# XiaRho/CMDA

Hardware: AMD Instinct MI355X
Metric: training images/sec (512x512 image+event, MiT-B5) (higher is better)
Workload: dtype bf16

## Files before the change

cmda_amd/csrc/batchnorm.hip:

```cpp
#include "common.h"

namespace {

constexpr int kRowUnroll = 4;
constexpr int kBnSlots = CMDA_BN_SLOTS;

template <typename T>
__global__ void bn_reduce_kernel(const T* __restrict__ x, float* __restrict__ ws, long M, int C, int rows_per_block) {
  __shared__ float red[2][4][64][4];
  const int cx = threadIdx.x & 63, ry = threadIdx.x >> 6;
  const int c = (blockIdx.x * 64 + cx) * 4;
  x += (long)blockIdx.z * M * C;
  ws += (long)blockIdx.z * (kBnSlots + 1) * 2 * C;
  const long r0 = (long)blockIdx.y * rows_per_block, r1 = min(M, r0 + rows_per_block);
  float s[4] = {0, 0, 0, 0}, q[4] = {0, 0, 0, 0};
  if (c < C) {
    float sh[4];
    ld4(x + c, sh);
    for (long r = r0 + ry; r < r1; r += 4 * kRowUnroll) {
      float v[kRowUnroll][4];
#pragma unroll
      for (int u = 0; u < kRowUnroll; ++u) {
        const long ru = r + 4 * u;
        ld4(x + (ru < r1 ? ru : r) * C + c, v[u]);
// ... 276 lines not shown
    for (int u = 0; u < kRowUnroll; ++u) {
      const long ru = r + 4 * u;
      if (ru >= r1) break;
#pragma unroll
      for (int j = 0; j < 4; ++j) {
        const float xh = (v[u][j] - mu[j]) * rs[j];
        float dj = d[u][j];
        if (relu && xh * g[j] + b[j] <= 0.f) dj = 0.f;
        v[u][j] = g[j] * rs[j] * (dj - a1[j] - xh * a2[j]);
      }
      st4(dx + ru * C + c, v[u]);
    }
  }
}

static inline int rows_per_block(long M, int gx) {
  int rpb = 512;
  while (rpb > 32 && (M + rpb - 1) / rpb * gx < 1024) rpb >>= 1;
  return rpb;
}
static inline int rows_per_block_apply(long M, int gx) {
  int rpb = 256;
  while (rpb > 16 && (M + rpb - 1) / rpb * gx < 2048) rpb >>= 1;
  return rpb;
}
}

extern "C" int64_t cmda_bn_ws_floats(int C) { return (int64_t)(kBnSlots + 1) * 2 * C; }

extern "C" int cmda_bn_train_fwd(const void* x, const float* gamma, const float* beta, void* y, float* mean, float* rstd,
                                 float* running_mean, float* running_var, float* ws, int64_t M, int C, float eps,
                                 float momentum, int relu, int ldy, int coff, int groups, const int* order, int ws_has_stats,
                                 int dtype, void* stream) {
  if (M <= 0 || C <= 0) return CMDA_OK;
  if ((C & 3) || (ldy & 3) || (coff & 3) || groups < 1 || groups > 8) return CMDA_ERR_SHAPE;
  BnOrder ord;
  for (int i = 0; i < 8; ++i) ord.g[i] = (order && i < groups) ? order[i] : i;
  unsigned seen = 0;
  for (int i = 0; i < groups; ++i) {
    if (ord.g[i] < 0 || ord.g[i] >= groups) return CMDA_ERR_SHAPE;
    seen |= 1u << ord.g[i];
  }
  if (ws_has_stats && seen != (1u << groups) - 1u) return CMDA_ERR_SHAPE;
  if (!ws_has_stats) cmda_zero_async(ws, sizeof(float) * (size_t)groups * (kBnSlots + 1) * 2 * C, stream);
  const int gx = (C / 4 + 63) / 64;
  const int rpb = rows_per_block(M * groups, gx);
  dim3 rgrid(gx, (unsigned)((M + rpb - 1) / rpb), groups);
  const int arpb = rows_per_block_apply(M * groups, gx);
  dim3 agrid(gx, (unsigned)((M + arpb - 1) / arpb), groups);
  CMDA_DISPATCH_DTYPE(dtype, {
    if (!ws_has_stats) CMDA_LAUNCH((bn_reduce_kernel<T>), rgrid, dim3(256), 0, stream, (const T*)x, ws, (long)M, C, rpb);
    CMDA_LAUNCH((bn_finalize_kernel<T>), dim3((C + 7) / 8), dim3(256), 0, stream, (const T*)x, ws, mean, rstd,
                running_mean, running_var, (long)M, C, eps, momentum, groups, ord, ws_has_stats);
    CMDA_LAUNCH((bn_apply_kernel<T>), agrid, dim3(256), 0, stream, (const T*)x, mean, rstd, gamma, beta, (T*)y + coff, (long)M,
                C, relu, ldy, 0, arpb);
  });
  CMDA_CHECK_LAUNCH();
}

extern "C" int cmda_bn_train_fwd2(const void* x, int x_dtype, const float* gamma, const float* beta, void* y, int y_dtype,
                                  float* mean, float* rstd, float* running_mean, float* running_var, float* ws, int64_t M, int C,
                                  float eps, float momentum, int relu, int ldy, int coff, int groups, const int* order,
                                  const float* res32, void* y2_bf16, int ws_has_stats, void* stream) {
  if (M <= 0 || C <= 0) return CMDA_OK;
  if ((C & 3) || (ldy & 3) || (coff & 3) || groups < 1 || groups > 8) return CMDA_ERR_SHAPE;
  if ((x_dtype != CMDA_F32 && x_dtype != CMDA_BF16) || (y_dtype != CMDA_F32 && y_dtype != CMDA_BF16)) return CMDA_ERR_DTYPE;
  BnOrder ord;
  for (int i = 0; i < 8; ++i) ord.g[i] = (order && i < groups) ? order[i] : i;
  unsigned seen = 0;
  for (int i = 0; i < groups; ++i) {
    if (ord.g[i] < 0 || ord.g[i] >= groups) return CMDA_ERR_SHAPE;
    seen |= 1u << ord.g[i];
  }
  if (ws_has_stats && seen != (1u << groups) - 1u) return CMDA_ERR_SHAPE;
  if (!ws_has_stats) cmda_zero_async(ws, sizeof(float) * (size_t)groups * (kBnSlots + 1) * 2 * C, stream);
  const int gx = (C / 4 + 63) / 64;
  const int rpb = rows_per_block(M * groups, gx);
  dim3 rgrid(gx, (unsigned)((M + rpb - 1) / rpb), groups);
  const int arpb = rows_per_block_apply(M * groups, gx);
  dim3 agrid(gx, (unsigned)((M + arpb - 1) / arpb), groups);
#define CMDA_BN2_APPLY(TX, TY)                                                                                                    \
  CMDA_LAUNCH((bn_apply2_kernel<TX, TY>), agrid, dim3(256), 0, stream, (const TX*)x, mean, rstd, gamma, beta, (TY*)y + coff,      \
              res32, (bf16_t*)y2_bf16, (long)M, C, relu, ldy, arpb)
  CMDA_DISPATCH_DTYPE(x_dtype, {
    if (!ws_has_stats) CMDA_LAUNCH((bn_reduce_kernel<T>), rgrid, dim3(256), 0, stream, (const T*)x, ws, (long)M, C, rpb);
    CMDA_LAUNCH((bn_finalize_kernel<T>), dim3((C + 7) / 8), dim3(256), 0, stream, (const T*)x, ws, mean, rstd,
                running_mean, running_var, (long)M, C, eps, momentum, groups, ord, ws_has_stats);
    if (y_dtype == CMDA_F32) CMDA_BN2_APPLY(T, float); else CMDA_BN2_APPLY(T, bf16_t);
  });
#undef CMDA_BN2_APPLY
  CMDA_CHECK_LAUNCH();
}

extern "C" int cmda_bn_apply(const void* x, const float* mean, const float* rstd, const float* gamma, const float* beta,
                             void* y, int64_t M, int C, int relu, int ldy, int coff, int dtype, void* stream) {
  if (M <= 0 || C <= 0) return CMDA_OK;
  if ((C & 3) || (ldy & 3) || (coff & 3)) return CMDA_ERR_SHAPE;
  const int gx = (C / 4 + 63) / 64;
  const int arpb = rows_per_block_apply(M, gx);
  dim3 agrid(gx, (unsigned)((M + arpb - 1) / arpb));
  CMDA_DISPATCH_DTYPE(dtype, CMDA_LAUNCH((bn_apply_kernel<T>), agrid, dim3(256), 0, stream, (const T*)x, mean, rstd, gamma,
                                         beta, (T*)y, (long)M, C, relu, ldy, coff, arpb));
  CMDA_CHECK_LAUNCH();
}

extern "C" int cmda_bn_train_bwd(const void* dy, const void* x, const float* mean, const float* rstd, const float* gamma,
                                 const float* beta, void* dx, float* dgamma, float* dbeta, float* ws, int64_t M, int C,
                                 int relu, int lddy, int coff, int groups, int dtype, void* stream) {
// ... 18 lines not shown
```

cmda_amd/csrc/gemm_pp.hip:

```cpp
#include "gemm_kernels.h"

namespace {

typedef __attribute__((ext_vector_type(16))) float f32x16;

#ifndef CMDA_EMU
static __device__ __forceinline__ f32x16 mfma_bf16_32x32x16(u16x8 a, u16x8 b, f32x16 c) {
  return __builtin_amdgcn_mfma_f32_32x32x16_bf16(__builtin_bit_cast(bfx8, a), __builtin_bit_cast(bfx8, b), c, 0, 0, 0);
}
static __device__ __forceinline__ void raw_barrier() { __builtin_amdgcn_s_barrier(); }
static __device__ __forceinline__ void sched_fence() { __builtin_amdgcn_sched_barrier(0); }
static __device__ __forceinline__ void prio(int hi) {
  if (hi) __builtin_amdgcn_s_setprio(1);
  else __builtin_amdgcn_s_setprio(0);
}
static __device__ __forceinline__ void wait_lds() { asm volatile("s_waitcnt lgkmcnt(0)" ::: "memory"); }
static __device__ __forceinline__ void wait_dma_lds() { asm volatile("s_waitcnt vmcnt(0) lgkmcnt(0)" ::: "memory"); }
#else
static inline f32x16 mfma_bf16_32x32x16(u16x8 a, u16x8 b, f32x16 c) {
  auto& w = emu::my_wave();
  const int l = emu::my_lane();
  for (int j = 0; j < 8; ++j) { w.fa[l][j] = bf2f(a[j]); w.fb[l][j] = bf2f(b[j]); }
  emu::wave_barrier();
  const int col = l & 31, h = l >> 5;
  f32x16 d = c;
  for (int r = 0; r < 16; ++r) {
    const int row = (r & 3) + 8 * (r >> 2) + 4 * h;
    float acc = d[r];
    for (int hh = 0; hh < 2; ++hh)
      for (int j = 0; j < 8; ++j) acc = fmaf(w.fa[32 * hh + row][j], w.fb[32 * hh + col][j], acc);
    d[r] = acc;
  }
  emu::wave_barrier();
  return d;
}
static inline void raw_barrier() { __syncthreads(); }
static inline void sched_fence() {}
static inline void prio(int) {}
static inline void wait_lds() {}
static inline void wait_dma_lds() { emu::wave_barrier(); }
#endif

#ifdef CMDA_PP_TIMING
__device__ unsigned long long g_pp_stamps[2 * 4 * 4 * 4];
#define PP_STAMP(i) do { if (lane == 0 && (wid & 3) == 0 && blockIdx.x == 7 && kt >= 8 && kt < 12) \
    g_pp_stamps[((grp * 4 + (kt - 8)) * 4 + q) * 4 + (i)] = __builtin_amdgcn_s_memtime(); } while (0)
#else
#define PP_STAMP(i) do { } while (0)
#endif

constexpr int PP_BM = 256, PP_BN = 256, PP_BK = 64, PP_NW = 8;
constexpr int PP_SZ = PP_BM * PP_BK;
constexpr int PP_PITCH_C = PP_BN + 8;
constexpr size_t PP_LDS = (size_t)PP_BM * PP_PITCH_C * 2;

template <int ACT>
static __device__ __forceinline__ float pp_act(float x) {
  if (ACT == 1) return fmaxf(x, 0.f);
  if (ACT == 2) return gelu_erf(x);
  if (ACT == 3) return tanhf(x);
  return x;
}

template <bool BKS, bool ACONV, bool FAST = false>
__global__ __launch_bounds__(512, 1) void gemm_pp_kernel(GemmParams p) {
  typedef bf16_t T;
  __shared__ __attribute__((aligned(1024))) char smem[PP_LDS];
  T* const sAbase = reinterpret_cast<T*>(smem);
  T* const sBbase = sAbase + 2 * PP_SZ;

  const int tid = threadIdx.x, lane = tid & 63;
#ifndef CMDA_EMU
  const int wid = __builtin_amdgcn_readfirstlane(tid >> 6);
#else
  const int wid = tid >> 6;
#endif
  const int grp = wid >> 2, wc = wid & 3;
  const int l31 = lane & 31, h = lane >> 5;

  const int tiles_n = (p.N + PP_BN - 1) / PP_BN;
  const int ntile = gridDim.x;
  int bt = blockIdx.x;
  {
    const int q = ntile / 8, rr = ntile % 8, xcd = bt % 8, loc = bt / 8;
    bt = (xcd < rr ? xcd * (q + 1) : rr * (q + 1) + (xcd - rr) * q) + loc;
  }
  long mt, nt;
  {
    constexpr int GM = 4;
    const int tiles_m = (int)((p.M + PP_BM - 1) / PP_BM);
    if (tiles_n >= 2 * GM && tiles_m >= GM) {
      const int gsz = GM * tiles_n, gid = bt / gsz, first = gid * GM;
      const int gm = min(tiles_m - first, GM), r = bt - gid * gsz;
      mt = first + r % gm;
      nt = r / gm;
    } else {
      mt = bt / tiles_n;
      nt = bt % tiles_n;
    }
  }
  const long m0 = mt * PP_BM, n0 = nt * PP_BN;
  const int z = blockIdx.z;
  const int batch = z / p.batch2, batch2 = z - batch * p.batch2;
  const int nkt = (p.K + PP_BK - 1) / PP_BK;
  const T* baseA = reinterpret_cast<const T*>(p.A.ptr) + (long)batch * p.A.batch_stride + (long)batch2 * p.A.batch2_stride;
  const T* baseB = reinterpret_cast<const T*>(p.B.ptr) + (long)batch * p.B.batch_stride + (long)batch2 * p.B.batch2_stride;

  DmaSrc<false, PP_BM, ACONV, PP_NW, 1, 64, DmaMode<false, ACONV, FAST>::value> dA;
  DmaSrc<BKS, PP_BN, false, PP_NW, 1, 64, DmaMode<BKS, false, FAST>::value> dB;
  dA.init(p.A, baseA, wid, lane, m0, 0);
  dB.init(p.B, baseB, wid, lane, n0, 0);
  bool cellA = false;
  auto piece = [&](int stage, int kt, int i) {
    if (i == 0) cellA = dA.cell_begin(kt, 0);
    if (i < 4) glds16(dA.get(p.A, baseA, i, kt, cellA), reinterpret_cast<char*>(sAbase + stage * PP_SZ) + (wid * 4 + i) * 1024);
    else glds16(dB.get(p.B, baseB, i - 4, kt, false), reinterpret_cast<char*>(sBbase + stage * PP_SZ) + (wid * 4 + (i - 4)) * 1024);
  };

  f32x16 acc[4][2];
#pragma unroll
  for (int i = 0; i < 4; ++i)
#pragma unroll
    for (int j = 0; j < 2; ++j)
#pragma unroll
      for (int r = 0; r < 16; ++r) acc[i][j][r] = 0.f;

  auto load_a = [&](const T* sA, int mh, u16x8 (&fa)[2][4]) {
#pragma unroll
    for (int i = 0; i < 2; ++i) {
      const int row = grp * 128 + (mh * 2 + i) * 32 + l31;
#pragma unroll
      for (int s = 0; s < 4; ++s) fa[i][s] = *reinterpret_cast<const u16x8*>(&sA[row * PP_BK + (((2 * s + h) ^ ((row >> 1) & 7)) << 3)]);
    }
  };
  auto load_b = [&](const T* sB, int nh, u16x8 (&fb)[4]) {
    if constexpr (!BKS) {
      const int row = wc * 64 + nh * 32 + l31;
#pragma unroll
      for (int s = 0; s < 4; ++s) fb[s] = *reinterpret_cast<const u16x8*>(&sB[row * PP_BK + (((2 * s + h) ^ ((row >> 1) & 7)) << 3)]);
    } else {
      const int gi = lane >> 4, li = lane & 15, q = li >> 2, pp = li & 3;
      const int colbase = wc * 64 + nh * 32 + 16 * (gi & 1);
      const int cidx = (colbase >> 3) + (pp >> 1), half = (pp & 1) << 2;
#pragma unroll
      for (int s = 0; s < 4; ++s) {
        const int k0 = 16 * s + 8 * (gi >> 1) + q, k1 = k0 + 4;
        const u16x4 lo = lds_read_tr16(&sB[k0 * PP_BN + ((cidx ^ (k0 & 7)) << 3) + half]);
        const u16x4 hi = lds_read_tr16(&sB[k1 * PP_BN + ((cidx ^ (k1 & 7)) << 3) + half]);
        fb[s] = u16x8{lo[0], lo[1], lo[2], lo[3], hi[0], hi[1], hi[2], hi[3]};
      }
    }
  };

#pragma unroll
  for (int i = 0; i < 8; ++i) piece(0, 0, i);
  wait_dma_lds();
  raw_barrier();
  if (grp == 1) raw_barrier();

  u16x8 fa[2][4], fb[2][4];
  for (int kt = 0; kt < nkt; ++kt) {
    const int st = kt & 1;
    const T* sA = sAbase + st * PP_SZ;
    const T* sB = sBbase + st * PP_SZ;
    const bool more = kt + 1 < nkt;
#pragma unroll
    for (int q = 0; q < 4; ++q) {
      const int mh = q >> 1, nh = (q == 1 || q == 2) ? 1 : 0;
      PP_STAMP(0);
      if (q == 0 || q == 2) load_a(sA, mh, fa);
      if (q < 2) load_b(sB, nh, fb[nh]);
      if (more) {
        if (q == 0) { piece(st ^ 1, kt + 1, 0); piece(st ^ 1, kt + 1, 4); }
        if (q == 1) { piece(st ^ 1, kt + 1, 1); piece(st ^ 1, kt + 1, 2); piece(st ^ 1, kt + 1, 5); piece(st ^ 1, kt + 1, 6); }
        if (q == 2) { piece(st ^ 1, kt + 1, 3); piece(st ^ 1, kt + 1, 7); }
      }
      if (q == 3 && grp == 1) wait_dma_lds();
      if (q == 3 && grp == 0) wait_lds();
      sched_fence();
      raw_barrier();
      wait_lds();
      PP_STAMP(1);
      sched_fence();
      prio(1);
#pragma unroll
      for (int s = 0; s < 4; ++s)
#pragma unroll
        for (int i = 0; i < 2; ++i) acc[mh * 2 + i][nh] = mfma_bf16_32x32x16(fb[nh][s], fa[i][s], acc[mh * 2 + i][nh]);
      prio(0);
      PP_STAMP(2);
      if (q == 3 && grp == 0) wait_dma_lds();
      sched_fence();
      raw_barrier();
      PP_STAMP(3);
    }
  }
  if (grp == 0) raw_barrier();
  __syncthreads();

  T* sC = reinterpret_cast<T*>(smem);
  const float alpha = p.alpha;
  const int act = p.act;
#pragma unroll
  for (int j = 0; j < 2; ++j)
#pragma unroll
    for (int rg = 0; rg < 4; ++rg) {
      const int nl = wc * 64 + j * 32 + 8 * rg + 4 * h;
      float bv[4] = {0.f, 0.f, 0.f, 0.f};
      if (p.bias) {
#pragma unroll
        for (int e = 0; e < 4; ++e)
          if (n0 + nl + e < p.N) bv[e] = p.bias[n0 + nl + e];
      }
#pragma unroll
      for (int i = 0; i < 4; ++i) {
        const int ml = grp * 128 + i * 32 + l31;
        float v[4];
#pragma unroll
        for (int e = 0; e < 4; ++e) v[e] = alpha * acc[i][j][rg * 4 + e] + bv[e];
        if (act == 1) {
#pragma unroll
          for (int e = 0; e < 4; ++e) v[e] = pp_act<1>(v[e]);
        } else if (act == 2) {
#pragma unroll
          for (int e = 0; e < 4; ++e) v[e] = pp_act<2>(v[e]);
        } else if (act == 3) {
#pragma unroll
          for (int e = 0; e < 4; ++e) v[e] = pp_act<3>(v[e]);
        }
        st4(&sC[ml * PP_PITCH_C + nl], v);
      }
    }
  __syncthreads();
  const long cb = (long)batch * p.c_batch_stride + (long)batch2 * p.c_batch2_stride;
  T* C = reinterpret_cast<T*>(p.C) + cb;
  const bool vec = p.c_vec_ok != 0 && (p.ldc & 7) == 0 && ((reinterpret_cast<uintptr_t>(C) & 15) == 0);
  const bool stats = p.colstats != nullptr;
  float cs[8] = {0.f, 0.f, 0.f, 0.f, 0.f, 0.f, 0.f, 0.f}, cq[8] = {0.f, 0.f, 0.f, 0.f, 0.f, 0.f, 0.f, 0.f};
#pragma unroll 4
  for (int it = 0; it < (PP_BM * PP_BN / 8) / 512; ++it) {
    const int idx = it * 512 + tid;
    const int row = idx >> 5, ch = idx & 31;
    const long m = m0 + row, n = n0 + ch * 8;
// ... 20 lines not shown
    }
  }
  if (stats) {
#pragma unroll
    for (int e = 0; e < 8; ++e) {
      cs[e] += __shfl_xor(cs[e], 32, 64);
      cq[e] += __shfl_xor(cq[e], 32, 64);
    }
    __syncthreads();
    float* scr = reinterpret_cast<float*>(smem);
    const int wv = tid >> 6, ln = tid & 63;
    if (ln < 32) {
#pragma unroll
      for (int e = 0; e < 8; ++e) {
        scr[wv * 2 * PP_BN + ln * 8 + e] = cs[e];
        scr[wv * 2 * PP_BN + PP_BN + ln * 8 + e] = cq[e];
      }
    }
    __syncthreads();
    static_assert(2 * PP_BN == 512, "one thread per (statistic, column)");
    const int col = tid & (PP_BN - 1);
    if (n0 + col < p.N) {
      float t = 0.f;
#pragma unroll
      for (int w = 0; w < 8; ++w) t += scr[w * 2 * PP_BN + tid];
      const long gidx = (unsigned)m0 / (unsigned)p.colstats_rows;
      const unsigned slot = (unsigned)(m0 >> 6) & (CMDA_BN_SLOTS - 1);
      atomicAdd(p.colstats + (gidx * (CMDA_BN_SLOTS + 1) + slot) * 2 * (long)p.N + (tid < PP_BN ? 0 : p.N) + n0 + col, t);
    }
  }
}

}

#ifdef CMDA_PP_TIMING
extern "C" int cmda_debug_pp_stamps(unsigned long long* host_out) {
  return hipMemcpyFromSymbol(host_out, HIP_SYMBOL(g_pp_stamps), sizeof(unsigned long long) * 128) == hipSuccess ? 0 : -3;
}
#endif

int cmda_gemm_pp_(const cmda_gemm_params_t& p, void* stream) {
  const long tiles = (long)((p.M + PP_BM - 1) / PP_BM) * ((p.N + PP_BN - 1) / PP_BN);
  const long zz = (long)p.batch * p.batch2;
  if (tiles > 0x7fffffffL || zz > 65535) return CMDA_ERR_SHAPE;
  const dim3 grid((unsigned)tiles, 1, (unsigned)zz), blk(512);
  const bool bks = p.b_kstrided != 0, ac = p.A.conv == 1;
  if (p.a_kstrided || p.B.conv == 1) return CMDA_ERR_UNSUPPORTED;
  const bool nofast = p.tile_hint > 0 && (p.tile_hint & 2048);
  typedef DmaSrc<false, PP_BM, false, PP_NW, 1, 64, 1> FA;
  typedef DmaSrc<false, PP_BM, true, PP_NW, 1, 64, 2> FAC;
  typedef DmaSrc<false, PP_BN, false, PP_NW, 1, 64, 1> FB;
  typedef DmaSrc<true, PP_BN, false, PP_NW, 1, 64, 1> FBK;
  if (!bks && !ac) {
    if (!nofast && FA::mode_ok(p.A, 1) && FB::mode_ok(p.B, 1)) CMDA_LAUNCH((gemm_pp_kernel<false, false, true>), grid, blk, 0, stream, p);
    else CMDA_LAUNCH((gemm_pp_kernel<false, false, false>), grid, blk, 0, stream, p);
  } else if (!bks && ac) {
    if (!nofast && FAC::mode_ok(p.A, 2) && FB::mode_ok(p.B, 1)) CMDA_LAUNCH((gemm_pp_kernel<false, true, true>), grid, blk, 0, stream, p);
    else CMDA_LAUNCH((gemm_pp_kernel<false, true, false>), grid, blk, 0, stream, p);
  } else if (bks && !ac) {
    if (!nofast && FA::mode_ok(p.A, 1) && FBK::mode_ok(p.B, 1)) CMDA_LAUNCH((gemm_pp_kernel<true, false, true>), grid, blk, 0, stream, p);
    else CMDA_LAUNCH((gemm_pp_kernel<true, false, false>), grid, blk, 0, stream, p);
  }
  else return CMDA_ERR_UNSUPPORTED;
  CMDA_CHECK_LAUNCH();
}
```

cmda_amd/decode_heads.py:

```python
import torch
import torch.nn as nn

from . import nn as K
from . import deferred, ops
from . import runtime as rt
from .registry import HEADS, LOSSES, build_loss


class ConvModule(nn.Module):

    def __init__(self, cin, cout, k, padding=0, dilation=1, groups=1, norm=True):
        super().__init__()
        self.conv = nn.Conv2d(cin, cout, k, padding=padding, dilation=dilation, groups=groups, bias=not norm)
        self.bn = nn.BatchNorm2d(cout) if norm else None
        nn.init.kaiming_normal_(self.conv.weight, a=0, mode='fan_out', nonlinearity='relu')
        if self.conv.bias is not None:
            nn.init.zeros_(self.conv.bias)
        self.k, self.padding, self.dilation, self.groups = k, padding, dilation, groups


class DepthwiseSeparableConvModule(nn.Module):
    def __init__(self, cin, cout, k, padding, dilation):
        super().__init__()
        self.depthwise_conv = ConvModule(cin, cin, k, padding=padding, dilation=dilation, groups=cin)
# ... 11 lines not shown
        return None
    return ops.bn_stats_ws(dev, groups, C)


def _bn_fwd(bn, x, y, M, C, relu, ldy=None, coff=0, groups=1, order=None, stats_ws=None):
    if bn.training:
        mean, rstd = ops.bn_train_fwd(x, bn.weight, bn.bias, y, bn.running_mean, bn.running_var, M // groups, C, bn.eps,
                                      bn.momentum, relu, ldy, coff, groups, order, stats_ws=stats_ws)
    else:
        mean, rstd = bn.running_mean, torch.rsqrt(bn.running_var + bn.eps)
        ops.bn_apply(x, mean, rstd, bn.weight, bn.bias, y, M, C, relu, ldy, coff)
        mean, rstd = mean.expand(groups, C).contiguous(), rstd.expand(groups, C).contiguous()
    return mean, rstd


def _bn_bwd(bn, dy, x, stats, M, C, relu, lddy=None, coff=0, groups=1):
    mean, rstd = stats
    return ops.bn_train_bwd(dy, x, mean, rstd, bn.weight, bn.bias, rt.grad(bn.weight), rt.grad(bn.bias), M // groups, C, relu,
                            lddy, coff, groups)


class ASPPWrapper(nn.Module):

    def __init__(self, in_channels, channels, sep, dilations, pool=False, norm_cfg=None, act_cfg=None,
                 align_corners=False, context_cfg=None):
        super().__init__()
        assert not pool and context_cfg is None, 'only the configuration CMDA uses is implemented'
        assert sep, 'CMDA uses the depthwise-separable ASPP'
        self.dilations = tuple(dilations)
        self.in_channels, self.channels = in_channels, channels
        mods = []
        for d in self.dilations:
            mods.append(ConvModule(in_channels, channels, 1) if d == 1 else
                        DepthwiseSeparableConvModule(in_channels, channels, 3, padding=d, dilation=d))
        self.aspp_modules = nn.ModuleList(mods)
        self.bottleneck = ConvModule(len(self.dilations) * channels, channels, 3, padding=1)

    def fwd(self, x, B, H, W, groups=1, order=None):
        M, Cin, Ch = B * H * W, self.in_channels, self.channels
        nb = len(self.dilations)
        cat = torch.empty(M, nb * Ch, dtype=rt.compute_dtype(), device=x.device)
        saved = []
        g = dict(groups=groups, order=order)
        for j, (d, m) in enumerate(zip(self.dilations, self.aspp_modules)):
            if d == 1:
                ws = _bn_stats_ws(m.bn, x.device, M, Ch, groups)
                z = K.linear_fwd(x, m.conv.weight, None, M, Cin, colstats=None if ws is None else (ws, M // groups))
                st = _bn_fwd(m.bn, z, cat, M, Ch, True, nb * Ch, j * Ch, stats_ws=ws, **g)
                saved.append((z, st))
            else:
                dwm, pwm = m.depthwise_conv, m.pointwise_conv
                ws = _bn_stats_ws(dwm.bn, x.device, M, Cin, groups) if (d >= 2 and B % groups == 0) else None
                u = ops.dwconv_fwd(x, rt.wdw(dwm.conv.weight), None, B, H, W, Cin, d, None, colstats=None if ws is None else (ws, B // groups))
                ub = torch.empty_like(u)
                st_u = _bn_fwd(dwm.bn, u, ub, M, Cin, True, stats_ws=ws, **g)
                ws = _bn_stats_ws(pwm.bn, x.device, M, Ch, groups)
                z = K.linear_fwd(ub, pwm.conv.weight, None, M, Cin, colstats=None if ws is None else (ws, M // groups))
                st_z = _bn_fwd(pwm.bn, z, cat, M, Ch, True, nb * Ch, j * Ch, stats_ws=ws, **g)
                saved.append((u, st_u, ub, z, st_z))
        ws = _bn_stats_ws(self.bottleneck.bn, x.device, M, Ch, groups)
        zb, _, _ = K.conv_fwd(cat, self.bottleneck.conv.weight, None, B, H, W, 1, 1, colstats=None if ws is None else (ws, M // groups))
        feat = torch.empty_like(zb)
        st_b = _bn_fwd(self.bottleneck.bn, zb, feat, M, Ch, True, stats_ws=ws, **g)
        return feat, (x, cat, saved, zb, st_b, groups)

    def bwd(self, sv, dfeat, B, H, W):
        x, cat, saved, zb, st_b, groups = sv
        M, Cin, Ch = B * H * W, self.in_channels, self.channels
        nb = len(self.dilations)
        dzb = _bn_bwd(self.bottleneck.bn, dfeat, zb, st_b, M, Ch, True, groups=groups)
        dcat = K.conv_bwd(dzb, cat, self.bottleneck.conv.weight, None, B, H, W, 1, 1)
        dx = torch.empty(M, Cin, dtype=rt.compute_dtype(), device=x.device)
        first = True
        for j, (d, m) in enumerate(zip(self.dilations, self.aspp_modules)):
            if d == 1:
                z, st = saved[j]
                dz = _bn_bwd(m.bn, dcat, z, st, M, Ch, True, nb * Ch, j * Ch, groups=groups)
                K.linear_bwd(dz, x, m.conv.weight, None, M, Cin, dx_out=dx, dx_beta=0.0 if first else 1.0)
            else:
                u, st_u, ub, z, st_z = saved[j]
                dwm, pwm = m.depthwise_conv, m.pointwise_conv
                dz = _bn_bwd(pwm.bn, dcat, z, st_z, M, Ch, True, nb * Ch, j * Ch, groups=groups)
                dub = K.linear_bwd(dz, ub, pwm.conv.weight, None, M, Cin)
                du = _bn_bwd(dwm.bn, dub, u, st_u, M, Cin, True, groups=groups)
                deferred.tail_defer(lambda du=du, gw=rt.grad(dwm.conv.weight).view(Cin, 9), d=d:
                                    ops.dwconv_bwd_weight(du, x, gw, None, B, H, W, Cin, d))
                ops.dwconv_bwd_data(du, rt.wdw(dwm.conv.weight), B, H, W, Cin, d, out=dx, accumulate=not first)
            first = False
        return dx


def build_layer(in_channels, out_channels, type, **kwargs):
    if type == 'id':
        return nn.Identity()
    if type == 'mlp':
        return MLP(input_dim=in_channels, embed_dim=out_channels)
    if type == 'aspp':
        return ASPPWrapper(in_channels=in_channels, channels=out_channels, **kwargs)
    raise NotImplementedError(type)


@LOSSES.register_module()
class CrossEntropyLoss(nn.Module):

    def __init__(self, use_sigmoid=False, use_mask=False, reduction='mean', class_weight=None, loss_weight=1.0):
        super().__init__()
        assert not use_sigmoid and not use_mask, 'only the softmax cross-entropy of configs/fusion/* is implemented'
        assert reduction == 'mean'
        self.use_sigmoid, self.use_mask, self.reduction = use_sigmoid, use_mask, reduction
        self.loss_weight, self.class_weight = loss_weight, class_weight


def ce_losses_fwd(logits, seg_label, seg_weight, ignore_index, loss_weight):
    B, _, H, W = seg_label.shape
    label = seg_label.view(B, H, W)
    wgt = seg_weight.float().contiguous() if seg_weight is not None else None
    acc, lse = ops.ce_upsample_fwd(logits, label, wgt, H, W, ignore_index)
    n = float(B * H * W)
    loss = acc[0] * (loss_weight / n)
    accuracy = acc[1:2] * (100.0 / n)
    return loss, accuracy, (logits, label, wgt, lse, H, W, n)


def ce_losses_bwd(saved, gscale, mul, ignore_index, loss_weight, out=None):
    logits, label, wgt, lse, H, W, n = saved
    return ops.ce_upsample_bwd(logits, label, wgt, lse, gscale, mul * loss_weight / n, H, W, ignore_index, out=out)


class _HeadBase(nn.Module):
    def __init__(self, in_channels, channels, *, num_classes, dropout_ratio=0.1, conv_cfg=None, norm_cfg=None,
                 act_cfg=dict(type='ReLU'), in_index=-1, input_transform=None,
                 loss_decode=dict(type='CrossEntropyLoss', use_sigmoid=False, loss_weight=1.0), decoder_params=None,
                 ignore_index=255, sampler=None, align_corners=False, init_cfg=None):
        super().__init__()
        assert input_transform == 'multiple_select' and sampler is None
        assert isinstance(in_channels, (list, tuple)) and isinstance(in_index, (list, tuple))
# ... 344 lines not shown
```

cmda_amd/nn.py:

```python
import os

import torch

from . import ops
from . import runtime as rt
from .ops import conv_view, plain_view


def linear_fwd(x, weight, bias, M, K, *, act=None, res=None, rowscale=None, rows_per_scale=1, out=None, ldc=None,
               c_offset=0, out_dtype=None, x_ld=None, x_off=0, colstats=None):
    N = weight.shape[0]
    if out is None:
        out = torch.empty(M, N, dtype=out_dtype or rt.compute_dtype(), device=x.device)
    ops.gemm(plain_view(x, M, K, ld=x_ld, offset=x_off), plain_view(rt.w(weight), N, K), out, M, N, K, dtype=rt.tag(),
             bias=bias, act=act, res=res, rowscale=rowscale, rows_per_scale=rows_per_scale, ldc=ldc, c_offset=c_offset, colstats=colstats)
    return out


def linear_bwd(dy, x, weight, bias, M, K, *, need_dx=True, dx_out=None, dx_beta=0.0, dy_ld=None, dy_off=0, x_ld=None,
               x_off=0):
    N = weight.shape[0]
    dyv_k = plain_view(dy, M, N, ld=dy_ld, offset=dy_off)
    xv = plain_view(x, M, K, ld=x_ld, offset=x_off)
    fused = (bias is not None and rt.tag() == 1 and dyv_k.vec_ok and xv.vec_ok and N % 8 == 0 and K % 8 == 0
             and (dy_ld or N) % 8 == 0 and (x_ld or K) % 8 == 0)
    fused = fused or (bias is not None and rt.tag() == 2 and dyv_k.vec_ok and xv.vec_ok and M % 32 == 0 and N % 4 == 0 and K % 4 == 0
                      and (dy_ld or N) % 4 == 0 and (x_ld or K) % 4 == 0 and ops.GEMM_TILE_HINT == 0)
    def wgrad():
        ops.gemm(dyv_k, xv, rt.grad(weight), N, K, M, a_kstrided=True, b_kstrided=True, dtype=rt.tag(), atomic=True,
                 splits=0, colsum=rt.grad(bias) if fused else None,
                 defer=True, keep=(dy, x))
        if bias is not None and not fused:
            ops.colsum(dy, rt.grad(bias), M, N, ld=dy_ld, offset=dy_off)
    rt.side('wgrad', wgrad, dy, x)
    if not need_dx:
        return None
    dx = dx_out if dx_out is not None else torch.empty(M, K, dtype=rt.compute_dtype(), device=dy.device)
    ops.gemm(dyv_k, plain_view(rt.w(weight), N, K), dx, M, K, N, b_kstrided=True, dtype=rt.tag(), beta=dx_beta)
    return dx


def conv_out_size(H, W, k, stride, pad, dil=1):
    return (H + 2 * pad - dil * (k - 1) - 1) // stride + 1, (W + 2 * pad - dil * (k - 1) - 1) // stride + 1


def conv_fwd(x, weight, bias, B, H, W, stride, pad, dil=1, *, act=None, out=None, reflect=0, ci_pad=0, colstats=None):
    Co, Ci, KH, KW = weight.shape
    Ci = max(Ci, ci_pad)
    OH, OW = conv_out_size(H, W, KH, stride, pad, dil)
    M, K = B * OH * OW, KH * KW * Ci
    if out is None:
        out = torch.empty(M, Co, dtype=rt.compute_dtype(), device=x.device)
    ops.gemm(conv_view(x, B, H, W, Ci, KH, KW, stride, pad, dil, OH=OH, OW=OW, reflect=reflect),
             plain_view(rt.wconv(weight, ci_pad=ci_pad), Co, K), out, M, Co, K, dtype=rt.tag(), bias=bias, act=act, colstats=colstats)
    return out, OH, OW


def conv_bwd(dy, x, weight, bias, B, H, W, stride, pad, dil=1, *, need_dx=True, dx_out=None, dx_beta=0.0, ci_pad=0):
    Co, Ci, KH, KW = weight.shape
    if ci_pad > Ci:
        assert not need_dx
        with ops.backward_scope():
            return _conv_bwd(dy, x, weight, bias, B, H, W, stride, pad, dil, need_dx=False, ci_pad=ci_pad)
    return _conv_bwd(dy, x, weight, bias, B, H, W, stride, pad, dil, need_dx=need_dx, dx_out=dx_out, dx_beta=dx_beta)


def _conv_bwd(dy, x, weight, bias, B, H, W, stride, pad, dil=1, *, need_dx=True, dx_out=None, dx_beta=0.0, ci_pad=0):
    Co, Ci, KH, KW = weight.shape
    Ci = max(Ci, ci_pad)
    OH, OW = conv_out_size(H, W, KH, stride, pad, dil)
    M, K = B * OH * OW, KH * KW * Ci
    def wgrad():
        dyv = plain_view(dy, M, Co)
        fused = (bias is not None and rt.tag() == 1 and dyv.vec_ok and Co % 8 == 0 and K % 8 == 0 and Ci % 8 == 0)
        shadow = ops.conv_grad_shadow(rt.grad(weight), ci_pad)
        if shadow is not None:
            ops.gemm(dyv, conv_view(x, B, H, W, Ci, KH, KW, stride, pad, dil, OH=OH, OW=OW), shadow, Co, K, M,
                     a_kstrided=True, b_kstrided=True, dtype=rt.tag(), atomic=True, splits=0,
                     colsum=rt.grad(bias) if fused else None, defer=True, keep=(dy, x))
        else:
            ops.gemm(dyv, conv_view(x, B, H, W, Ci, KH, KW, stride, pad, dil, OH=OH, OW=OW), rt.grad(weight), Co, K, M,
                     a_kstrided=True, b_kstrided=True, dtype=rt.tag(), atomic=True, splits=0, c_perm=(Ci, KH * KW),
                     colsum=rt.grad(bias) if fused else None)
        if bias is not None and not fused:
            ops.colsum(dy, rt.grad(bias), M, Co)
    rt.side('wgrad', wgrad, dy, x)
    if not need_dx:
        return None
    dx = dx_out if dx_out is not None else torch.empty(B * H * W, Ci, dtype=rt.compute_dtype(), device=dy.device)
    if KH == stride and pad == 0 and dil == 1 and H % stride == 0 and W % stride == 0:
        ops.gemm(plain_view(dy, M, Co), plain_view(rt.wconv(weight), Co, K), dx, M, K, Co, b_kstrided=True, dtype=rt.tag(),
                 beta=dx_beta, c_patch=(OW, KH, KW * Ci))
# ... 138 lines not shown
```

cmda_amd/ops.py:

```python
import ctypes
import os

import numpy as np
import torch

from . import _lib as L
from . import deferred as D
from ._lib import BF16, F32, GemmParams, View, c_f32, c_i32, c_i64, call, check_dev, dtype_tag, ptr, stream_of

_ESIZE = {torch.float32: 4, torch.bfloat16: 2}


def _chunk(t):
    return 16 // _ESIZE[t.dtype]


def plain_view(t, rows, cols, ld=None, batch_stride=0, offset=0, batch2_stride=0):
    ld = cols if ld is None else ld
    es = _ESIZE[t.dtype]
    ch = 16 // es
    base = t.data_ptr() + offset * es
    vec_ok = int(base % 16 == 0 and ld % ch == 0 and batch_stride % ch == 0 and batch2_stride % ch == 0)
    v = View(ptr=base, ld=ld, R=rows, Cc=cols, batch_stride=batch_stride, batch2_stride=batch2_stride, conv=0,
             vec_ok=vec_ok,
# ... 519 lines not shown
         c_i32(C), c_i32(dil), dtype_tag(x), stream_of(x))
    return dz


def dwconv_gelu_bwd_fused(x, w, bias, da, dw, dbias, B, H, W, C, dil=1):
    check_dev(x, w, bias, da, dw, dbias)
    dz = torch.empty_like(x)
    call('cmda_dwconv3x3_gelu_bwd_fused', ptr(x), ptr(w), ptr(bias), ptr(da), ptr(dz), ptr(dw), ptr(dbias), c_i32(B), c_i32(H),
         c_i32(W), c_i32(C), c_i32(dil), dtype_tag(x), stream_of(x))
    return dz


def dwconv_bwd_data(dy, w, B, H, W, C, dil=1, out=None, accumulate=False):
    check_dev(dy, w, out)
    dx = torch.empty_like(dy) if out is None else out
    call('cmda_dwconv3x3_bwd_data', ptr(dy), ptr(w), ptr(dx), c_i32(B), c_i32(H), c_i32(W), c_i32(C), c_i32(dil),
         c_i32(int(accumulate)), dtype_tag(dy), stream_of(dy))
    return dx


def dwconv_bwd_weight(dz, x, dw, dbias, B, H, W, C, dil=1):
    check_dev(dz, x, dw, dbias)
    call('cmda_dwconv3x3_bwd_weight', ptr(dz), ptr(x), ptr(dw), ptr(dbias), c_i32(B), c_i32(H), c_i32(W), c_i32(C),
         c_i32(dil), dtype_tag(x), stream_of(x))


def bilinear_fwd(x, y, B, IH, IW, OH, OW, C, ldy=None, coff=0):
    check_dev(x, y)
    call('cmda_bilinear_fwd', ptr(x), ptr(y), c_i32(B), c_i32(IH), c_i32(IW), c_i32(OH), c_i32(OW), c_i32(C),
         c_i32(C if ldy is None else ldy), c_i32(coff), dtype_tag(x), stream_of(x))
    return y


def bilinear_bwd(dy, dx, B, IH, IW, OH, OW, C, ldy=None, coff=0):
    check_dev(dy, dx)
    call('cmda_bilinear_bwd', ptr(dy), ptr(dx), c_i32(B), c_i32(IH), c_i32(IW), c_i32(OH), c_i32(OW), c_i32(C),
         c_i32(C if ldy is None else ldy), c_i32(coff), dtype_tag(dy), stream_of(dy))
    return dx


BN_FUSED_STATS = os.environ.get('CMDA_BN_FUSED_STATS', '1') != '0'
def bn_stats_ws(device, groups, C):
    if not BN_FUSED_STATS:
        return None
    need = groups * int(L.lib().cmda_bn_ws_floats(C))
    ws = D.workspace('bn', device, need, make_in_capture=False)
    return None if ws is None else ws[:need]


def colstats_ok(rows_per_group, N):
    return BN_FUSED_STATS and rows_per_group > 0 and rows_per_group % 256 == 0 and N % 4 == 0


def bn_train_fwd(x, gamma, beta, y, running_mean, running_var, M, C, eps, momentum, relu, ldy=None, coff=0, groups=1, order=None,
                 stats_ws=None):
    check_dev(x, gamma, beta, y, running_mean, running_var, stats_ws)
    mean = torch.empty(groups, C, dtype=torch.float32, device=x.device)
    rstd = torch.empty(groups, C, dtype=torch.float32, device=x.device)
    ws = stats_ws if stats_ws is not None else torch.empty(groups * L.lib().cmda_bn_ws_floats(C), dtype=torch.float32, device=x.device)
    order_c = (ctypes.c_int * groups)(*order) if order is not None else None
    call('cmda_bn_train_fwd', ptr(x), ptr(gamma), ptr(beta), ptr(y), ptr(mean), ptr(rstd), ptr(running_mean),
         ptr(running_var), ptr(ws), c_i64(M), c_i32(C), c_f32(eps), c_f32(momentum), c_i32(int(relu)),
         c_i32(C if ldy is None else ldy), c_i32(coff), c_i32(groups), order_c, c_i32(int(stats_ws is not None)), dtype_tag(x), stream_of(x))
    return mean, rstd


def bn_train_fwd2(x, gamma, beta, y, M, C, eps, relu, groups=1, res32=None, y2=None, ldy=None, coff=0, stats_ws=None):
    check_dev(x, gamma, beta, y, res32, y2, stats_ws)
    assert res32 is None or res32.dtype == torch.float32
    assert y2 is None or y2.dtype == torch.bfloat16
    mean = torch.empty(groups, C, dtype=torch.float32, device=x.device)
    rstd = torch.empty(groups, C, dtype=torch.float32, device=x.device)
    ws = stats_ws if stats_ws is not None else torch.empty(groups * L.lib().cmda_bn_ws_floats(C), dtype=torch.float32, device=x.device)
    call('cmda_bn_train_fwd2', ptr(x), dtype_tag(x), ptr(gamma), ptr(beta), ptr(y), dtype_tag(y), ptr(mean), ptr(rstd), None, None,
         ptr(ws), c_i64(M), c_i32(C), c_f32(eps), c_f32(0.0), c_i32(int(relu)), c_i32(C if ldy is None else ldy), c_i32(coff),
         c_i32(groups), None, ptr(res32), ptr(y2), c_i32(int(stats_ws is not None)), stream_of(x))
    return mean, rstd


def bn_apply(x, mean, rstd, gamma, beta, y, M, C, relu, ldy=None, coff=0):
    check_dev(x, mean, rstd, gamma, beta, y)
    call('cmda_bn_apply', ptr(x), ptr(mean), ptr(rstd), ptr(gamma), ptr(beta), ptr(y), c_i64(M), c_i32(C),
         c_i32(int(relu)), c_i32(C if ldy is None else ldy), c_i32(coff), dtype_tag(x), stream_of(x))


def bn_train_bwd(dy, x, mean, rstd, gamma, beta, dgamma, dbeta, M, C, relu, lddy=None, coff=0, groups=1):
    check_dev(dy, x, mean, rstd, gamma, beta, dgamma, dbeta)
    dx = torch.empty_like(x)
    ws = torch.empty(groups * L.lib().cmda_bn_ws_floats(C), dtype=torch.float32, device=x.device)
    call('cmda_bn_train_bwd', ptr(dy), ptr(x), ptr(mean), ptr(rstd), ptr(gamma), ptr(beta), ptr(dx), ptr(dgamma),
         ptr(dbeta), ptr(ws), c_i64(M), c_i32(C), c_i32(int(relu)), c_i32(C if lddy is None else lddy), c_i32(coff),
         c_i32(groups), dtype_tag(x), stream_of(x))
    return dx


def ce_upsample_fwd(logits, label, weight, H, W, ignore_index=255, acc=None):
    check_dev(logits, label, weight, acc)
    B, h, w, nc = logits.shape
    lse = torch.empty(B, H, W, dtype=torch.float32, device=logits.device)
    if acc is None:
        acc = torch.zeros(2, dtype=torch.float32, device=logits.device)
    call('cmda_ce_upsample_fwd', ptr(logits), ptr(label), ptr(weight), ptr(lse), ptr(acc), c_i32(B), c_i32(h), c_i32(w),
         c_i32(H), c_i32(W), c_i32(nc), c_i32(ignore_index), stream_of(logits))
    return acc, lse


# ... 196 lines not shown
```

include/cmda_hip.h:

```cpp
#ifndef CMDA_HIP_H_
#define CMDA_HIP_H_
#include <stdint.h>

#ifdef __cplusplus
extern "C" {
#endif

#define CMDA_OK 0
#define CMDA_ERR_SHAPE -1
#define CMDA_ERR_DTYPE -2
#define CMDA_ERR_HIP -3
#define CMDA_ERR_UNSUPPORTED -4

#define CMDA_F32 0
#define CMDA_BF16 1
#define CMDA_F32X3 2

int cmda_abi_version(void);

typedef struct cmda_view_t {
  const void* ptr;
  int64_t ld;
  int64_t R, Cc;
  int64_t batch_stride;
  int64_t batch2_stride;
  int32_t conv;
  int32_t H, W, C;
  int32_t OH, OW;
  int32_t KH, KW, stride, pad, dil;
  int32_t in_dil;
  int32_t reflect;
  int32_t vec_ok;
} cmda_view_t;

typedef struct cmda_gemm_params_t {
  cmda_view_t A, B;
  int32_t a_kstrided;
  int32_t b_kstrided;
  void* C;
  int64_t ldc, c_batch_stride, c_batch2_stride;
  int32_t M, N, K, batch, batch2, splits;
  float alpha, beta;
  const float* bias;
  int32_t act;
  const void* res;
  int64_t ldres, res_batch_stride, res_batch2_stride;
  const float* rowscale;
  int32_t rows_per_scale;
  int32_t out_f32;
  int32_t atomic;
  int32_t dtype;
  int32_t c_vec_ok;
  float* colsum;
  int32_t c_patch_ow, c_patch_kh, c_patch_kwci;
  int32_t tile_hint;
  int32_t c_perm_ci, c_perm_cells;
  int32_t res_f32;
  int32_t colstats_rows;
  float* colstats;
} cmda_gemm_params_t;

int cmda_gemm(const cmda_gemm_params_t* p, void* stream);


int cmda_conv_co1(const void* x, const void* w, const float* bias, float* out, int B, int H, int W, int C, int K, int pad,
    int reflect, int act, int dtype, void* stream);
int cmda_conv_co3(const void* x, const void* w, const float* bias, const float* scale, const float* shift, float* out, int B, int H,
    int W, int C, int K, int pad, int reflect, int act, int dtype, void* stream);

int64_t cmda_gemm_grouped_ws_bytes(const cmda_gemm_params_t* params, int n);
int cmda_gemm_grouped(const cmda_gemm_params_t* params, int n, void* ws_host, void* ws_dev, int64_t ws_bytes, int upload, void* stream);

int cmda_layernorm_fwd(const void* x, const float* gamma, const float* beta, void* y, float* mean, float* rstd,
    int64_t rows, int C, float eps, int dtype, void* stream);
int64_t cmda_layernorm_bwd_ws_floats(int64_t rows, int C);
int cmda_layernorm_bwd(const void* dy, const void* x, const float* gamma, const float* mean, const float* rstd, const void* dres,
    void* dx, float* dgamma, float* dbeta, float* ws, int64_t rows, int C, const float* out_scale, int64_t rows_per_scale,
    void* dx_scaled, int dtype, void* stream);
int cmda_layernorm_fwd2(const void* x, int x_dtype, const float* gamma, const float* beta, void* y, int y_dtype, float* mean, float* rstd,
    int64_t rows, int C, float eps, void* stream);
int cmda_layernorm_bwd2(const void* dy, const void* x, int x_dtype, const float* gamma, const float* mean, const float* rstd,
    const void* dres, void* dx, float* dgamma, float* dbeta, float* ws, int64_t rows, int C, const float* out_scale,
    int64_t rows_per_scale, void* dx_scaled, int dtype, void* stream);
int cmda_layernorm_fold_batch(const void* desc, int n, int max_c, void* stream);
int cmda_layernorm_slots(void);

int cmda_softmax_fwd(void* s, int64_t rows, int L, float alpha, int dtype, void* stream);
int cmda_softmax_bwd(const void* p, void* dp, int64_t rows, int L, float alpha, int dtype, void* stream);

int cmda_attention_fwd(const void* q, const void* kv, void* o, int B, int N, int Nk, int heads, int C, float scale,
    int dtype, void* stream);
int64_t cmda_attention_bwd_ws_floats(int B, int N, int heads);
int cmda_attention_bwd_direct(int B, int N, int Nk, int heads);
int cmda_attention_bwd(const void* q, const void* kv, const void* d_o, void* dq, float* dkv32, void* dkv16, float* stats, int B,
    int N, int Nk, int heads, int C, float scale, int dtype, void* stream);
int cmda_attention_fwd_x3(const float* q, const void* kv_hi, const void* kv_lo, float* o, int B, int N, int Nk, int heads, int C,
    float scale, void* stream);
int cmda_attention_bwd_x3(const float* q, const void* kv_hi, const void* kv_lo, const float* d_o, float* dq, float* dkv32,
    float* dkv_direct, float* stats, int B, int N, int Nk, int heads, int C, float scale, void* stream);

int cmda_dwconv3x3_fwd(const void* x, const float* w, const float* bias, void* y, int B, int H, int W, int C, int dil,
    int act, int dtype, void* stream);
int cmda_dwconv3x3_fwd_stats(const void* x, const float* w, const float* bias, void* y, int B, int H, int W, int C, int dil,
    float* colstats, int imgs_per_group, int dtype, void* stream);
int cmda_dwconv3x3_gelu_bwd_prep(const void* x, const float* w, const float* bias, const void* da, void* dz, int B,
    int H, int W, int C, int dil, int dtype, void* stream);
int cmda_dwconv3x3_bwd_data(const void* dy, const float* w, void* dx, int B, int H, int W, int C, int dil, int
    accumulate, int dtype, void* stream);
int cmda_dwconv3x3_bwd_weight(const void* dz, const void* x, float* dw, float* dbias, int B, int H, int W, int C, int
    dil, int dtype, void* stream);
int cmda_dwconv3x3_gelu_bwd_fused(const void* x, const float* w, const float* bias, const void* da, void* dz, float* dw,
    float* dbias, int B, int H, int W, int C, int dil, int dtype, void* stream);

int cmda_bilinear_fwd(const void* x, void* y, int B, int IH, int IW, int OH, int OW, int C, int ldy, int coff, int
    dtype, void* stream);
int cmda_bilinear_bwd(const void* dy, void* dx, int B, int IH, int IW, int OH, int OW, int C, int ldy, int coff, int
// ... 94 lines not shown
```

Baseline: 39.33.

## Fuse BatchNorm+ReLU into pointwise GEMM A-operand load in decode head

In the decode head's depthwise-separable convs, the BN+ReLU apply on the depthwise output is folded into the pointwise GEMM: the gemm_pp kernel gets a BNA variant that rewrites each A tile in LDS with normalize/affine/ReLU before the MFMAs. This skips the separate bn_apply kernel and the materialized ub tensor in forward. Backward recomputes ub lazily in a deferred weight-grad task, with dgrad computed without dW. It adds LDS for per-channel params and extra per-k-step ALU/LDS work plus barriers in the GEMM inner loop, and recomputation in backward.

```diff
diff --git a/cmda_amd/csrc/batchnorm.hip b/cmda_amd/csrc/batchnorm.hip
--- a/cmda_amd/csrc/batchnorm.hip
+++ b/cmda_amd/csrc/batchnorm.hip
@@ -352,8 +352,9 @@
     if (!ws_has_stats) CMDA_LAUNCH((bn_reduce_kernel<T>), rgrid, dim3(256), 0, stream, (const T*)x, ws, (long)M, C, rpb);
     CMDA_LAUNCH((bn_finalize_kernel<T>), dim3((C + 7) / 8), dim3(256), 0, stream, (const T*)x, ws, mean, rstd,
                 running_mean, running_var, (long)M, C, eps, momentum, groups, ord, ws_has_stats);
-    CMDA_LAUNCH((bn_apply_kernel<T>), agrid, dim3(256), 0, stream, (const T*)x, mean, rstd, gamma, beta, (T*)y + coff, (long)M,
-                C, relu, ldy, 0, arpb);
+    if (y)
+      CMDA_LAUNCH((bn_apply_kernel<T>), agrid, dim3(256), 0, stream, (const T*)x, mean, rstd, gamma, beta, (T*)y + coff, (long)M,
+                  C, relu, ldy, 0, arpb);
   });
   CMDA_CHECK_LAUNCH();
 }
diff --git a/cmda_amd/csrc/gemm_pp.hip b/cmda_amd/csrc/gemm_pp.hip
--- a/cmda_amd/csrc/gemm_pp.hip
+++ b/cmda_amd/csrc/gemm_pp.hip
@@ -53,6 +53,15 @@
 constexpr int PP_SZ = PP_BM * PP_BK;
 constexpr int PP_PITCH_C = PP_BN + 8;
 constexpr size_t PP_LDS = (size_t)PP_BM * PP_PITCH_C * 2;
+constexpr int PP_BNA_KMAX = 1024;
+
+struct PpBnA {
+  const float* mean;
+  const float* rstd;
+  const float* gamma;
+  const float* beta;
+  long rows_per_group;
+};
 
 template <int ACT>
 static __device__ __forceinline__ float pp_act(float x) {
@@ -62,10 +71,11 @@
   return x;
 }
 
-template <bool BKS, bool ACONV, bool FAST = false>
-__global__ __launch_bounds__(512, 1) void gemm_pp_kernel(GemmParams p) {
+template <bool BKS, bool ACONV, bool FAST = false, bool BNA = false>
+__global__ __launch_bounds__(512, 1) void gemm_pp_kernel(GemmParams p, PpBnA bn) {
+  static_assert(!BNA || (!BKS && !ACONV), "BatchNorm on the operand load: plain K-contiguous A and B");
   typedef bf16_t T;
-  __shared__ __attribute__((aligned(1024))) char smem[PP_LDS];
+  __shared__ __attribute__((aligned(1024))) char smem[PP_LDS + (BNA ? 4 * PP_BNA_KMAX * sizeof(float) : 0)];
   T* const sAbase = reinterpret_cast<T*>(smem);
   T* const sBbase = sAbase + 2 * PP_SZ;
 
@@ -116,6 +126,44 @@
     if (i < 4) glds16(dA.get(p.A, baseA, i, kt, cellA), reinterpret_cast<char*>(sAbase + stage * PP_SZ) + (wid * 4 + i) * 1024);
     else glds16(dB.get(p.B, baseB, i - 4, kt, false), reinterpret_cast<char*>(sBbase + stage * PP_SZ) + (wid * 4 + (i - 4)) * 1024);
   };
+  float* const sP = reinterpret_cast<float*>(smem + PP_LDS);
+  const int bc = lane & 7;
+  if constexpr (BNA) {
+    const long g = m0 / bn.rows_per_group;
+    for (int k = tid; k < p.K; k += 512) {
+      sP[k] = bn.mean[g * p.K + k];
+      sP[PP_BNA_KMAX + k] = bn.rstd[g * p.K + k];
+      sP[2 * PP_BNA_KMAX + k] = bn.gamma[k];
+      sP[3 * PP_BNA_KMAX + k] = bn.beta[k];
+    }
+    __syncthreads();
+  }
+  auto a_fix = [&](int stage, int kt) {
+    T* const sA = sAbase + stage * PP_SZ;
+    const int k = kt * PP_BK + bc * 8;
+    f32x4 pm[2], pr[2], pg[2], pb[2];
+#pragma unroll
+    for (int h2 = 0; h2 < 2; ++h2) {
+      pm[h2] = *reinterpret_cast<const f32x4*>(&sP[k + 4 * h2]);
+      pr[h2] = *reinterpret_cast<const f32x4*>(&sP[PP_BNA_KMAX + k + 4 * h2]);
+      pg[h2] = *reinterpret_cast<const f32x4*>(&sP[2 * PP_BNA_KMAX + k + 4 * h2]);
+      pb[h2] = *reinterpret_cast<const f32x4*>(&sP[3 * PP_BNA_KMAX + k + 4 * h2]);
+    }
+#pragma unroll
+    for (int i = 0; i < 4; ++i) {
+      const int line = wid * 32 + i * 8 + (lane >> 3);
+      u16x8* const slot = reinterpret_cast<u16x8*>(&sA[line * PP_BK + ((bc ^ ((line >> 1) & 7)) << 3)]);
+      const u16x8 x = *slot;
+      u16x8 o;
+#pragma unroll
+      for (int e = 0; e < 8; ++e) {
+        float v = (bf2f(x[e]) - pm[e >> 2][e & 3]) * pr[e >> 2][e & 3] * pg[e >> 2][e & 3] + pb[e >> 2][e & 3];
+        v = fmaxf(v, 0.f);
+        o[e] = f2bf(v);
+      }
+      *slot = o;
+    }
+  };
 
   f32x16 acc[4][2];
 #pragma unroll
@@ -155,6 +203,10 @@
 #pragma unroll
   for (int i = 0; i < 8; ++i) piece(0, 0, i);
   wait_dma_lds();
+  if constexpr (BNA) {
+    a_fix(0, 0);
+    wait_lds();
+  }
   raw_barrier();
   if (grp == 1) raw_barrier();
 
@@ -189,6 +241,13 @@
         for (int i = 0; i < 2; ++i) acc[mh * 2 + i][nh] = mfma_bf16_32x32x16(fb[nh][s], fa[i][s], acc[mh * 2 + i][nh]);
       prio(0);
       PP_STAMP(2);
+      if constexpr (BNA) {
+        if (q == 3 && more) {
+          if (grp == 0) wait_dma_lds();
+          a_fix(st ^ 1, kt + 1);
+          wait_lds();
+        }
+      }
       if (q == 3 && grp == 0) wait_dma_lds();
       sched_fence();
       raw_barrier();
@@ -315,15 +374,55 @@
   typedef DmaSrc<false, PP_BN, false, PP_NW, 1, 64, 1> FB;
   typedef DmaSrc<true, PP_BN, false, PP_NW, 1, 64, 1> FBK;
   if (!bks && !ac) {
-    if (!nofast && FA::mode_ok(p.A, 1) && FB::mode_ok(p.B, 1)) CMDA_LAUNCH((gemm_pp_kernel<false, false, true>), grid, blk, 0, stream, p);
-    else CMDA_LAUNCH((gemm_pp_kernel<false, false, false>), grid, blk, 0, stream, p);
+    if (!nofast && FA::mode_ok(p.A, 1) && FB::mode_ok(p.B, 1)) CMDA_LAUNCH((gemm_pp_kernel<false, false, true>), grid, blk, 0, stream, p, PpBnA{});
+    else CMDA_LAUNCH((gemm_pp_kernel<false, false, false>), grid, blk, 0, stream, p, PpBnA{});
   } else if (!bks && ac) {
-    if (!nofast && FAC::mode_ok(p.A, 2) && FB::mode_ok(p.B, 1)) CMDA_LAUNCH((gemm_pp_kernel<false, true, true>), grid, blk, 0, stream, p);
-    else CMDA_LAUNCH((gemm_pp_kernel<false, true, false>), grid, blk, 0, stream, p);
+    if (!nofast && FAC::mode_ok(p.A, 2) && FB::mode_ok(p.B, 1)) CMDA_LAUNCH((gemm_pp_kernel<false, true, true>), grid, blk, 0, stream, p, PpBnA{});
+    else CMDA_LAUNCH((gemm_pp_kernel<false, true, false>), grid, blk, 0, stream, p, PpBnA{});
   } else if (bks && !ac) {
-    if (!nofast && FA::mode_ok(p.A, 1) && FBK::mode_ok(p.B, 1)) CMDA_LAUNCH((gemm_pp_kernel<true, false, true>), grid, blk, 0, stream, p);
-    else CMDA_LAUNCH((gemm_pp_kernel<true, false, false>), grid, blk, 0, stream, p);
+    if (!nofast && FA::mode_ok(p.A, 1) && FBK::mode_ok(p.B, 1)) CMDA_LAUNCH((gemm_pp_kernel<true, false, true>), grid, blk, 0, stream, p, PpBnA{});
+    else CMDA_LAUNCH((gemm_pp_kernel<true, false, false>), grid, blk, 0, stream, p, PpBnA{});
   }
   else return CMDA_ERR_UNSUPPORTED;
   CMDA_CHECK_LAUNCH();
 }
+
+extern "C" int cmda_gemm_bnrelu_pw(const void* u, const void* w, void* z, const float* mean, const float* rstd, const float* gamma,
+                                   const float* beta, int64_t M, int N, int K, int64_t rows_per_group, float* colstats, int dtype,
+                                   void* stream) {
+  if (dtype != CMDA_BF16) return CMDA_ERR_DTYPE;
+  if (M <= 0) return CMDA_OK;
+  if (N != PP_BN || K < PP_BK || K % PP_BK || K > PP_BNA_KMAX || M % PP_BM || M > 0x7fffffffL || rows_per_group <= 0 || rows_per_group % PP_BM ||
+      M % rows_per_group)
+    return CMDA_ERR_SHAPE;
+  auto a16 = [](const void* q) { return (reinterpret_cast<uintptr_t>(q) & 15) == 0; };
+  if (!a16(u) || !a16(w) || !a16(z) || !a16(mean) || !a16(rstd) || !a16(gamma) || !a16(beta)) return CMDA_ERR_SHAPE;
+  cmda_gemm_params_t p{};
+  p.A.ptr = u;
+  p.A.ld = K;
+  p.A.R = M;
+  p.A.Cc = K;
+  p.A.vec_ok = 1;
+  p.B.ptr = w;
+  p.B.ld = K;
+  p.B.R = N;
+  p.B.Cc = K;
+  p.B.vec_ok = 1;
+  p.C = z;
+  p.ldc = N;
+  p.M = (int)M;
+  p.N = N;
+  p.K = K;
+  p.batch = p.batch2 = p.splits = 1;
+  p.alpha = 1.f;
+  p.dtype = CMDA_BF16;
+  p.c_vec_ok = 1;
+  p.colstats = colstats;
+  p.colstats_rows = (int)rows_per_group;
+  const PpBnA bn{mean, rstd, gamma, beta, (long)rows_per_group};
+  const dim3 grid((unsigned)(M / PP_BM)), blk(512);
+  typedef DmaSrc<false, PP_BN, false, PP_NW, 1, 64, 1> FB;
+  if (FB::mode_ok(p.B, 1)) CMDA_LAUNCH((gemm_pp_kernel<false, false, true, true>), grid, blk, 0, stream, p, bn);
+  else CMDA_LAUNCH((gemm_pp_kernel<false, false, false, true>), grid, blk, 0, stream, p, bn);
+  CMDA_CHECK_LAUNCH();
+}
diff --git a/cmda_amd/decode_heads.py b/cmda_amd/decode_heads.py
--- a/cmda_amd/decode_heads.py
+++ b/cmda_amd/decode_heads.py
@@ -87,10 +87,15 @@
                 dwm, pwm = m.depthwise_conv, m.pointwise_conv
                 ws = _bn_stats_ws(dwm.bn, x.device, M, Cin, groups) if (d >= 2 and B % groups == 0) else None
                 u = ops.dwconv_fwd(x, rt.wdw(dwm.conv.weight), None, B, H, W, Cin, d, None, colstats=None if ws is None else (ws, B // groups))
-                ub = torch.empty_like(u)
+                fused = dwm.bn.training and ops.bnrelu_pw_ok(u, M, groups, Cin, Ch)
+                ub = None if fused else torch.empty_like(u)
                 st_u = _bn_fwd(dwm.bn, u, ub, M, Cin, True, stats_ws=ws, **g)
                 ws = _bn_stats_ws(pwm.bn, x.device, M, Ch, groups)
-                z = K.linear_fwd(ub, pwm.conv.weight, None, M, Cin, colstats=None if ws is None else (ws, M // groups))
+                if fused:
+                    z = ops.gemm_bnrelu_pw(u, rt.w(pwm.conv.weight), st_u[0], st_u[1], dwm.bn.weight, dwm.bn.bias, M, Cin, M // groups,
+                                           colstats=ws)
+                else:
+                    z = K.linear_fwd(ub, pwm.conv.weight, None, M, Cin, colstats=None if ws is None else (ws, M // groups))
                 st_z = _bn_fwd(pwm.bn, z, cat, M, Ch, True, nb * Ch, j * Ch, stats_ws=ws, **g)
                 saved.append((u, st_u, ub, z, st_z))
         ws = _bn_stats_ws(self.bottleneck.bn, x.device, M, Ch, groups)
@@ -116,7 +121,21 @@
                 u, st_u, ub, z, st_z = saved[j]
                 dwm, pwm = m.depthwise_conv, m.pointwise_conv
                 dz = _bn_bwd(pwm.bn, dcat, z, st_z, M, Ch, True, nb * Ch, j * Ch, groups=groups)
-                dub = K.linear_bwd(dz, ub, pwm.conv.weight, None, M, Cin)
+                if ub is not None:
+                    dub = K.linear_bwd(dz, ub, pwm.conv.weight, None, M, Cin)
+                else:
+                    dub = K.linear_bwd(dz, None, pwm.conv.weight, None, M, Cin, need_dw=False)
+                    key = deferred._QUEUE_KEY
+
+                    def pw_wgrad(dz=dz, u=u, st_u=st_u, bn=dwm.bn, weight=pwm.conv.weight, key=key):
+                        ub = torch.empty_like(u)
+                        Mg = M // groups
+                        for gi in range(groups):
+                            ops.bn_apply(u[gi * Mg:(gi + 1) * Mg], st_u[0][gi], st_u[1][gi], bn.weight, bn.bias, ub[gi * Mg:(gi + 1) * Mg],
+                                         Mg, Cin, True)
+                        with deferred.queue_under(key):
+                            K.linear_bwd(dz, ub, weight, None, M, Cin, need_dx=False)
+                    deferred.tail_defer(pw_wgrad)
                 du = _bn_bwd(dwm.bn, dub, u, st_u, M, Cin, True, groups=groups)
                 deferred.tail_defer(lambda du=du, gw=rt.grad(dwm.conv.weight).view(Cin, 9), d=d:
                                     ops.dwconv_bwd_weight(du, x, gw, None, B, H, W, Cin, d))
diff --git a/cmda_amd/nn.py b/cmda_amd/nn.py
--- a/cmda_amd/nn.py
+++ b/cmda_amd/nn.py
@@ -18,9 +18,19 @@
 
 
 def linear_bwd(dy, x, weight, bias, M, K, *, need_dx=True, dx_out=None, dx_beta=0.0, dy_ld=None, dy_off=0, x_ld=None,
-               x_off=0):
+               x_off=0, need_dw=True):
     N = weight.shape[0]
     dyv_k = plain_view(dy, M, N, ld=dy_ld, offset=dy_off)
+    if need_dw:
+        _linear_wgrad(dy, x, weight, bias, M, K, N, dyv_k, dy_ld, dy_off, x_ld, x_off)
+    if not need_dx:
+        return None
+    dx = dx_out if dx_out is not None else torch.empty(M, K, dtype=rt.compute_dtype(), device=dy.device)
+    ops.gemm(dyv_k, plain_view(rt.w(weight), N, K), dx, M, K, N, b_kstrided=True, dtype=rt.tag(), beta=dx_beta)
+    return dx
+
+
+def _linear_wgrad(dy, x, weight, bias, M, K, N, dyv_k, dy_ld, dy_off, x_ld, x_off):
     xv = plain_view(x, M, K, ld=x_ld, offset=x_off)
     fused = (bias is not None and rt.tag() == 1 and dyv_k.vec_ok and xv.vec_ok and N % 8 == 0 and K % 8 == 0
              and (dy_ld or N) % 8 == 0 and (x_ld or K) % 8 == 0)
@@ -33,11 +43,6 @@
         if bias is not None and not fused:
             ops.colsum(dy, rt.grad(bias), M, N, ld=dy_ld, offset=dy_off)
     rt.side('wgrad', wgrad, dy, x)
-    if not need_dx:
-        return None
-    dx = dx_out if dx_out is not None else torch.empty(M, K, dtype=rt.compute_dtype(), device=dy.device)
-    ops.gemm(dyv_k, plain_view(rt.w(weight), N, K), dx, M, K, N, b_kstrided=True, dtype=rt.tag(), beta=dx_beta)
-    return dx
 
 
 def conv_out_size(H, W, k, stride, pad, dil=1):
diff --git a/cmda_amd/ops.py b/cmda_amd/ops.py
--- a/cmda_amd/ops.py
+++ b/cmda_amd/ops.py
@@ -595,6 +595,23 @@
     return BN_FUSED_STATS and rows_per_group > 0 and rows_per_group % 256 == 0 and N % 4 == 0
 
 
+HEAD_PW = os.environ.get('CMDA_HEAD_PW', '1') != '0'
+
+
+def bnrelu_pw_ok(u, M, groups, K, N):
+    return (HEAD_PW and u.dtype == torch.bfloat16 and N == 256 and K % 64 == 0 and 64 <= K <= 1024 and M % groups == 0 and
+            (M // groups) % 256 == 0)
+
+
+def gemm_bnrelu_pw(u, w, mean, rstd, gamma, beta, M, K, rows_per_group, colstats=None):
+    check_dev(u, w, mean, rstd, gamma, beta, colstats)
+    N = w.shape[0]
+    z = torch.empty(M, N, dtype=u.dtype, device=u.device)
+    call('cmda_gemm_bnrelu_pw', ptr(u), ptr(w), ptr(z), ptr(mean), ptr(rstd), ptr(gamma), ptr(beta), c_i64(M), c_i32(N), c_i32(K),
+         c_i64(rows_per_group), ptr(colstats), dtype_tag(u), stream_of(u))
+    return z
+
+
 def bn_train_fwd(x, gamma, beta, y, running_mean, running_var, M, C, eps, momentum, relu, ldy=None, coff=0, groups=1, order=None,
                  stats_ws=None):
     check_dev(x, gamma, beta, y, running_mean, running_var, stats_ws)
diff --git a/include/cmda_hip.h b/include/cmda_hip.h
--- a/include/cmda_hip.h
+++ b/include/cmda_hip.h
@@ -62,6 +62,9 @@
 
 int cmda_gemm(const cmda_gemm_params_t* p, void* stream);
 
+int cmda_gemm_bnrelu_pw(const void* u, const void* w, void* z, const float* mean, const float* rstd, const float* gamma,
+    const float* beta, int64_t M, int N, int K, int64_t rows_per_group, float* colstats, int dtype, void* stream);
+
 
 int cmda_conv_co1(const void* x, const void* w, const float* bias, float* out, int B, int H, int W, int C, int K, int pad,
     int reflect, int act, int dtype, void* stream);
```

Result: no change. 39.39, median of 6 (+0.2%).
